# amazon-science/tubelet-transformer

Measured on AMD Instinct MI355X. Metric: clips/sec (TubeR CSN-152 AVA2.1 training step fwd+bwd+clip+AdamW, 32x256x340 clips; whole job), higher is better.
Workload: dtype bf16; 1 GPU; TubeR_CSN152_AVA21 train step, 2 clips/GPU of 3x32x256x340, dropout on, random-init name-hashed weights; global_batch=2, parallelism=dp1, launch_mode=hipgraph, lib_md5=ed8e0d92b699

## Files before the change

### include/tuber_hip.h

```cpp
#ifndef TUBER_HIP_H
#define TUBER_HIP_H

#ifdef __cplusplus
extern "C" {
#endif

typedef struct ihipStream_t* hipStream_t;

typedef struct TuberClipDesc {
    long long src_off;
    int H, W;
    int y1, x1, h, w;
    int flip, jitter;
    int hue, sat, val;
    int pad_;
} TuberClipDesc;

int tuber_attn_fwd(const void* Q, const long* mq, const void* K, const long* mk, const void* V, const long* mv, void* O, const long* mo, float* lse, const void* key_padding_mask, int B, int H, int Lq, int Lk, float scale, float pdrop, const void* seed_ptr, unsigned long long salt, hipStream_t stream);

int tuber_attn_bwd(const void* Q, const long* mq, const void* K, const long* mk, const void* V, const long* mv, const void* O, const long* mo, const float* lse, const void* key_padding_mask, const void* dO, const long* mdo, void* dQ, const long* mdq, void* dK, const long* mdk, void* dV, const long* mdv, float* delta, int B, int H, int Lq, int Lk, float scale, float pdrop, const void* seed_ptr, unsigned long long salt, hipStream_t stream);

int tuber_attn_wide_fwd(const void* q, const void* kv, void* o, int NQ, int HW, int T, float pdrop, const void* seed_ptr, unsigned long long salt, hipStream_t stream);

int tuber_attn_wide_bwd(const void* q, const void* kv, const void* dO, void* dq, void* dkv, int NQ, int HW, int T, float pdrop, const void* seed_ptr, unsigned long long salt, hipStream_t stream);
// ... 16 lines not shown

const char* tuber_comm_last_error(void);

int tuber_comm_unique_id(void* id128);

int tuber_comm_init(const void* id128, int nranks, int rank, int device, void** comm_out);

int tuber_comm_init_timeout(const void* id128, int nranks, int rank, int device, int timeout_ms, void** comm_out);

int tuber_comm_count(void* comm, int* count_out, int* rank_out);

int tuber_comm_allreduce_sum(void* comm, void* buf, long count, int dtype, hipStream_t stream);

int tuber_comm_allreduce_sum_multi(void* comm, void* const* ptrs, const long* counts, int n, int dtype, hipStream_t stream);

int tuber_comm_destroy(void* comm);

int tuber_conv1_bwd_slabs(long M);

int tuber_conv1_bwd_supported(int cin, int p);

int tuber_conv1_bwd_fused(const void* dz1, const void* c1, const float* cA, const float* cB, const float* cC, const void* w1t, long ldw, const void* R, const void* X, const void* Cm, const void* Cd, void* out, float* st0, float* st1, float* st2, float* slab, long M, hipStream_t stream);

int tuber_conv4_bwd_slabs(long M);

int tuber_conv4_bwd_supported(int c4, int p);

int tuber_conv4_bwd_fused(const void* dz, const void* c4, const void* c3, const void* w4t, long ldw, const float* cA, const float* cB, const float* cC, const float* sc3, const float* sh3, void* dz3, float* st0, float* st1, float* slab, long M, hipStream_t stream);

int tuber_criterion_cost(const float* logits, const float* logits_b, const float* boxes, const float* tboxes, const float* tlabels, const int* tcount, int L, int B, int Q, int C, int Tmax, int ava, float w_class, float w_bbox, float w_giou, float* cost, hipStream_t stream);

int tuber_criterion_loss(const float* logits, const float* logits_b, const float* boxes, const float* tboxes, const float* tlabels, const int* tcount, const int* match, int L, int B, int Q, int C, int Tmax, int ava, float eos, float pos_weight, float* losses, float* g_logits, float* g_logits_b, float* g_bbox, float* g_giou, hipStream_t stream);

int tuber_criterion_scale(const float* g, const float* g_logits, const float* g_logits_b, const float* g_bbox, const float* g_giou, int L, long nl, long nb, long nx, float* gl, float* gb, float* gx, hipStream_t stream);

int tuber_weighted_sum(const float* a, const float* w, int n, float* out, const float* gout, float* out_g, hipStream_t stream);

int tuber_lsap_device(const float* cost, const int* tcount, int* match, int L, int B, int Q, int Tmax, hipStream_t stream);

int tuber_class_error(const float* logits, const int* match, const float* tlabels, int B, int Q, int C, int Tmax, int ava, float* out, hipStream_t stream);

int tuber_targets_pack_max(void);

int tuber_targets_pack(const void* const* boxes, const void* const* labels, const int* sizes, int B, int Tmax, int C, int ava, float* tboxes, float* tlabels, int* tcount, hipStream_t stream);

int tuber_mask_resize(const void* mask, void* out, int B, int H, int W, int h, int w, hipStream_t stream);

int tuber_decoder_coop_supported(int d_model, int nhead, int dim_ff, int batch, int num_queries, int num_layers);

int tuber_decoder_coop_ptrs_per_layer(void);

int tuber_decoder_coop_fwd(const void* const* layer_ptrs, const unsigned long long* layer_salts, int num_layers, const void* qpos, const float* norm_weight, const float* norm_bias, void* hs, const void* kpm, int B, int Q, int Lm, float pdrop, float pattn, const void* seed_ptr, void* sync, hipStream_t stream);

int tuber_dwconv_fwd_stat_rows(int N, int To, int Ho, int Wo);

int tuber_dwconv_bwd_data_stat_rows(int N, int Ti, int Hi, int Wi);

int tuber_dwconv_bwd_weight_blocks(int N, int To, int Ho, int Wo);

int tuber_dwconv_fwd(const void* x, const float* sc, const float* sh, const float* w, void* out, float* st0, float* st1, int N, int Ti, int Hi, int Wi, int To, int Ho, int Wo, int C, int st, int ss, hipStream_t stream);

int tuber_dwconv_bwd_data(const void* gout, const float* w, const void* x, const float* sc, const float* sh, void* dz, float* st0, float* st1, int N, int Ti, int Hi, int Wi, int To, int Ho, int Wo, int C, int st, int ss, hipStream_t stream);

int tuber_dw_wgrad_reduce(const float* partial, float* dw, int R, int C, int accumulate, hipStream_t stream);

int tuber_dwconv_bwd_weight(const void* gout, const void* x, const float* sc, const float* sh, float* partial, float* dw, int accumulate, int N, int Ti, int Hi, int Wi, int To, int Ho, int Wo, int C, int st, int ss, hipStream_t stream);

int tuber_dwconv_tile_blocks(int N, int T, int H, int W, int C);

int tuber_dwconv_tile_wgrad_blocks(int N, int T, int H, int W, int C);

int tuber_dwconv_tile_fwd(const void* x, const float* sc, const float* sh, const float* w, void* out, float* st0, float* st1, int N, int T, int H, int W, int C, hipStream_t stream);

int tuber_dwconv_tile_fwd_bn(const void* x, const float* pst0, const float* pst1, int R, float count, const float* gamma, const float* beta, float* rmean, float* rvar, long long* nbt, float momentum, float eps, float* scale, float* shift, float* mean, float* invstd, const float* w, void* out, float* st0, float* st1, int N, int T, int H, int W, int C, hipStream_t stream);

int tuber_dwconv_tile_fwd_bn_ex(const void* x, const float* pst0, const float* pst1, int R, float count, const float* gamma, const float* beta, float* rmean, float* rvar, long long* nbt, float momentum, float eps, float* scale, float* shift, float* mean, float* invstd, const float* w, void* out, float* st0, float* st1, int N, int T, int H, int W, int C, hipStream_t stream);

int tuber_dwconv_tile_bwd_data(const void* gout, const float* w, const void* x, const float* sc, const float* sh, void* dz, float* st0, float* st1, int N, int T, int H, int W, int C, hipStream_t stream);

int tuber_dwconv_tile_bwd_weight(const void* gout, const void* x, const float* sc, const float* sh, float* partial, float* dw, int accumulate, int N, int T, int H, int W, int C, hipStream_t stream);

int tuber_dwconv_tile_bwd_data_bn(const void* dzu, const void* xu, const float* bst0, const float* bst1, int R, float count, const float* gamma, const float* mean, const float* invstd, float* dgamma, float* dbeta, const float* w, const void* x, const float* sc, const float* sh, void* dz, float* st0, float* st1, int N, int T, int H, int W, int C, hipStream_t stream);

int tuber_dwconv_tile_bwd_weight_bn(const void* dzu, const void* xu, const float* bst0, const float* bst1, int R, float count, const float* gamma, const float* mean, const float* invstd, const void* x, const float* sc, const float* sh, float* partial, float* dw, int accumulate, int N, int T, int H, int W, int C, hipStream_t stream);

int tuber_dwconv_tile_bwd_both_bn(const void* dzu, const void* xu, const float* bst0, const float* bst1, int R, float count, const float* gamma, const float* mean, const float* invstd, float* dgamma, float* dbeta, const float* w, const void* x, const float* sc, const float* sh, void* dz, float* st0, float* st1, float* partial, int N, int T, int H, int W, int C, hipStream_t stream);

int tuber_dwconv_tile_bwd_data_bn_frozen(const void* dzu, const float* bst0, const float* bst1, int R, const float* gamma, const float* mean, const float* invstd, float* dgamma, float* dbeta, const float* w, const void* x, const float* sc, const float* sh, void* dz, float* st0, float* st1, int N, int T, int H, int W, int C, hipStream_t stream);

int tuber_dwconv_tile_bwd_weight_bn_frozen(const void* dzu, const float* gamma, const float* mean, const float* invstd, const void* x, const float* sc, const float* sh, float* partial, float* dw, int accumulate, int N, int T, int H, int W, int C, hipStream_t stream);

int tuber_dwconv_tile_bwd_both_bn_frozen(const void* dzu, const float* bst0, const float* bst1, int R, const float* gamma, const float* mean, const float* invstd, float* dgamma, float* dbeta, const float* w, const void* x, const float* sc, const float* sh, void* dz, float* st0, float* st1, float* partial, int N, int T, int H, int W, int C, hipStream_t stream);

int tuber_cast_f32_bf16(const float* src, void* dst, long n, hipStream_t stream);

int tuber_cast_bf16_f32_scale(const void* src, float* dst, long n, float scale, hipStream_t stream);

int tuber_cast_transpose(const float* W, void* WT, int R, int C, int ldt, hipStream_t stream);

int tuber_rows_gather_sum(const void* in, void* out, int A, int B, int C, int D, long sa, long sb, long sc, long sd, int E, float mul, hipStream_t stream);

int tuber_temporal_max_fwd(const void* x, void* out, void* arg, int B, int T, long hw, int E, hipStream_t stream);

int tuber_temporal_max_bwd(const void* g, const void* arg, void* dx, int B, int T, long hw, int E, hipStream_t stream);

int tuber_axpby(const void* a, const void* b, void* out, long n, float alpha, float beta, hipStream_t stream);
// ... 189 lines not shown
```

### tubelet_transformer_amd/ab.py

```python
import contextlib
import os

KNOWN = {
    "no_wgrad_groups": "one tuber_gemm_tn launch per weight-gradient GEMM instead of the grouped launches (engine.WgradQueue)",
    "immediate_reduce": "second-stage reductions of the weight-gradient partials per call instead of the deferred tuber_multi_reduce",
    "no_join_fusion": "stand-alone block_out_bwd instead of the join backward in the conv1 data-gradient GEMM's epilogue",
    "no_fresh_reduce": "tuber_multi_reduce always reads the gradient window it reduces into (out += sum) instead of overwriting the windows zero_grad has just cleared",
    "no_join_mask": "the join backward reads the lower block's output y for its ReLU mask instead of the bit field tuber_block_out_fwd_mask writes (bit-identical gradients)",
    "no_strided_join_fusion": "gemm + rows_scatter_add + block_out_bwd at the stage boundaries instead of the join GEMM with the strided residual",
    "no_ds_join_fusion": "stand-alone block_out_bwd for the first block of every stage (the join kernels take identity-block joins only)",
    "no_bn_bwd_fa": "BatchNorm backward as finalize + apply launches everywhere (no one-launch form)",
    "no_bn_bwd_fa_after_reduce": "no one-launch BatchNorm backward behind the first-stage row reduction (layer1 / layer2)",
    "no_bn1_in_dw_fwd": "stand-alone tuber_bn_finalize for bn1 instead of finalising it inside the stride-1 depthwise forward kernel",
    "no_bn3_in_dw": "stand-alone bn_bwd_fa for bn3 instead of forming it inside the depthwise backward kernels",
    "no_dw_bwd_one_launch": "depthwise data and weight gradient of a stride-1 block as two launches",
    "no_conv4_bwd_fused": "layer1's conv4 backward on the separate BatchNorm / GEMM kernels",
    "no_conv1_bwd_fused": "layer1's conv1 backward on the separate BatchNorm / GEMM kernels",
    "no_blockout_conv1": "layer1's residual join and the next conv1 as two launches",
    "no_entry_conv": "conv1 and the projection conv of layer1's first block as two GEMMs",
    "no_proj_bwd_fused": "layer1's projection-shortcut backward on the separate kernels",
    "no_stem_bn_in_wgrad": "stand-alone bn_bwd_apply for the stem instead of forming it inside the stem weight-gradient kernel",
    "dw_register_tiled": "the register-tiled depthwise kernels (used for the strided blocks) for every block",
    "no_ln_bwd_fusion": "LayerNorm backward and the data-gradient GEMM of the linear in front of it as two launches (no tuber_ln_bwd_dx)",
    "no_in_proj_dx2": "the few-row data gradients of the decoder (in-projection: x and query_pos; linear1) as tuber_gemm_nt launches instead of tuber_rows_dx2",
    "no_decoder_coop": "the DETR decoder stack as its ~80 separate launches instead of the one cooperative launch (csrc/decoder_coop.hip)",
    "eager_step": "train_tuber_detection without the captured hipGraph step",
    "eval_bf16_stream": "eval forward with the residual streams (block outputs, LayerNorm outputs) stored in bf16 like the training path, instead of the fp32 "
                        "streams of the eval precision mode (round 6; also TUBER_EVAL_PRECISION=bf16_stream)",
    "no_eval_conv4_join": "eval precision mode with conv4 and the residual join of an identity block as two launches (tuber_gemm_nt + tuber_block_out_fwd_f32) "
                          "instead of the join in the GEMM epilogue (tuber_gemm_nt_bn_out; bit-identical outputs)",
    "eval_bf16_decoder": "eval precision mode without the fp32 decoder / heads (csrc/eval_f32.hip): the decoder on the bf16 launch chain with fp32 LayerNorm streams only",
}


def _parse(text):
    names = {t.strip().lower() for t in (text or "").replace(";", ",").split(",") if t.strip()}
    bad = sorted(names - set(KNOWN))
    if bad:
        raise ValueError("TUBER_AB: unknown switch(es) %s; known: %s" % (bad, sorted(KNOWN)))
    return names


_active = _parse(os.environ.get("TUBER_AB"))


def on(name):
    if name not in KNOWN:
        raise KeyError(name)
    return name in _active


def active():
    return sorted(_active)


def eval_fp32_stream():
    return not on("eval_bf16_stream") and os.environ.get("TUBER_EVAL_PRECISION", "fp32_stream") != "bf16_stream"


def eval_class_f32():
    return eval_fp32_stream() and os.environ.get("TUBER_EVAL_PRECISION") == "fp32_class"


@contextlib.contextmanager
def override(*names):
    global _active
    old = _active
    _active = _parse(",".join(names))
    try:
        yield
    finally:
        _active = old
```

### tubelet_transformer_amd/backbone.py

```python
import operator
from typing import NamedTuple

import torch
from torch import nn

from . import ab, lib

BN_EPS = 1e-3
BN_MOM = 0.1
BF = torch.bfloat16
CMAX = 2048
_MOMENTUM = operator.attrgetter("momentum")
_TRAINING = operator.attrgetter("training")


class ResNeXtBottleneck(nn.Module):

    def __init__(self, in_planes, planes, stride=1, temporal_stride=1, down_sample=None, expansion=2):
        super().__init__()
        self.expansion = expansion
        self.conv1 = nn.Conv3d(in_planes, planes, kernel_size=1, bias=False)
        self.bn1 = nn.BatchNorm3d(planes, eps=BN_EPS, momentum=BN_MOM)
        self.conv3 = nn.Conv3d(planes, planes, kernel_size=3, bias=False, stride=(temporal_stride, stride, stride),
                               padding=1, groups=planes)
# ... 27 lines not shown
            self.sigmoid = nn.Sigmoid()
        self._runner = None

    @staticmethod
    def _make_layer(in_planes, planes, blocks, stride, temporal_stride, expansion=4):
        ds = nn.Sequential(
            nn.Conv3d(in_planes, planes * expansion, kernel_size=1, stride=(temporal_stride, stride, stride), bias=False),
            nn.BatchNorm3d(planes * expansion, eps=BN_EPS, momentum=BN_MOM))
        layers = [ResNeXtBottleneck(in_planes, planes, stride, temporal_stride, ds, expansion)]
        for _ in range(1, blocks):
            layers.append(ResNeXtBottleneck(planes * expansion, planes, expansion=expansion))
        return nn.Sequential(*layers)

    def forward(self, x):
        raise RuntimeError("ResNeXt runs through tubelet_transformer_amd.tuber.DETR (needs the model's ParamStore)")


def build_CSN(cfg):
    name = cfg.CONFIG.MODEL.BACKBONE_NAME
    if name == "CSN-152":
        m = ResNeXt([3, 8, 36, 3], cfg.CONFIG.DATA.NUM_CLASSES, cfg.CONFIG.MODEL.LAST_STRIDE, with_out_fc=False)
    elif name == "CSN-50":
        m = ResNeXt([3, 4, 6, 3], cfg.CONFIG.DATA.NUM_CLASSES, cfg.CONFIG.MODEL.LAST_STRIDE, with_out_fc=True)
    elif name == "CSN-TEST":
        m = ResNeXt([2, 2, 2, 2], cfg.CONFIG.DATA.NUM_CLASSES, cfg.CONFIG.MODEL.LAST_STRIDE, with_out_fc=False)
    else:
        raise ValueError("unsupported BACKBONE_NAME %r (CSN-50 / CSN-152)" % name)
    if cfg.CONFIG.MODEL.PRETRAINED:
        from .checkpoint import load_csn_mat
        load_csn_mat(m, cfg.CONFIG.MODEL.PRETRAIN_BACKBONE_DIR, name)
    return m


class _BN:
    __slots__ = ("idx", "mod", "C", "gamma", "beta", "rmean", "rvar", "nbt", "dgamma", "dbeta", "scale", "shift", "mean", "invstd",
                 "cA", "cB", "cC")


class _Block:
    __slots__ = ("cin", "p", "st", "ss", "ds", "off0", "stage", "first", "mod", "w1", "g1", "w1t", "ld1t", "w3", "g3", "w4", "g4", "w4t", "ld4t",
                 "bn1", "bn3", "bn4", "wd", "gd", "wdt", "lddt", "bnd")

    @property
    def strided(self):
        return self.st != 1 or self.ss != 1

    @property
    def c4(self):
        return 4 * self.p


_Saved = NamedTuple("_Saved", [(n, object) for n in ("x", "c1", "c3", "c4", "cd", "y", "geom", "ymask")])
_SavedStem = NamedTuple("_SavedStem", [(n, object) for n in ("clips", "c0", "arg", "geom")])


def _rows(B, geom):
    Ti, Hi, Wi, To, Ho, Wo = geom
    return B * Ti * Hi * Wi, B * To * Ho * Wo


class CSNRunner:

    def __init__(self, body: ResNeXt, prefix: str, store):
        self.body, self.store = body, store
        dev = store.device
        self.dev = dev
        bns = [m for m in body.modules() if isinstance(m, nn.BatchNorm3d)]
        self.scratch = torch.zeros(len(bns), 7, CMAX, dtype=torch.float32, device=dev)
        self._bn_index = {}
        self._bn_rows = []
        self.blocks = []
        self.cut_stages = (3,)
        self.split_hook = None
        self.last_y32 = None
        sp = self.scratch.data_ptr()

        def mk_bn(mod_prefix, mod):
            b = _BN()
            i = len(self._bn_index)
            self._bn_index[mod_prefix] = i
            b.idx, b.mod = i, mod
            f, g = store.flat.data_ptr(), store.gflat.data_ptr()
            ow, ob = store.offsets[mod_prefix + ".weight"], store.offsets[mod_prefix + ".bias"]
            b.C = mod.num_features
            b.gamma, b.beta = f + 4 * ow, f + 4 * ob
            b.dgamma, b.dbeta = g + 4 * ow, g + 4 * ob
            b.rmean, b.rvar, b.nbt = mod.running_mean.data_ptr(), mod.running_var.data_ptr(), mod.num_batches_tracked.data_ptr()
            base = sp + 4 * i * 7 * CMAX
            b.scale, b.shift, b.mean, b.invstd, b.cA, b.cB, b.cC = (base + 4 * k * CMAX for k in range(7))
            self._bn_rows.append((i, b))
            return b

        def wptr(name):
            o = store.offsets[name]
            return store.shadow.data_ptr() + 2 * o, store.flat.data_ptr() + 4 * o, store.gflat.data_ptr() + 4 * o

        def tptr(name):
            toff, N, K, ldt = store.tinfo[name]
            return store.tshadow.data_ptr() + 2 * toff, ldt

        self.stem_w32 = store.flat.data_ptr() + 4 * store.offsets[prefix + "conv1.weight"]
        self.stem_g = store.gflat.data_ptr() + 4 * store.offsets[prefix + "conv1.weight"]
        self.stem_wpad = torch.zeros(64, 512, dtype=BF, device=dev)
        self.stem_bn = mk_bn(prefix + "bn1", body.bn1)
        for li in range(1, 5):
            layer = getattr(body, "layer%d" % li)
# ... 453 lines not shown
            if fuse4:
                S4 = lib.query("tuber_conv4_bwd_slabs", Mout)
                part4, acc4 = self.store.partial("c4f", S4 * C4 * P)
                lib.call("tuber_conv4_bwd_fused", dz, sv.c4, c3, d.w4t, d.ld4t, b4.cA, b4.cB, b4.cC, b3.scale, b3.shift,
                         dz3, s0, s1, part4, Mout)
                self._slab_reduce(part4, acc4, d.g4, C4 * P, S4)
            else:
                lib.gemm_nt(dc4, C4, d.w4t, d.ld4t, dz3, P, Mout, P, C4, epi=2, stat0=s0, stat1=s1, Cm=c3, ldcm=P, m_scale=b3.scale, m_shift=b3.shift)
            frz3 = b3.idx in self._frozen
            sfx = "_frozen" if frz3 else ""
            if fuse3 and frz3:
                bs0, bs1, bR = (None, None, 0) if not f["bn3"] else (s0, s1, R3) if R3 <= self._fa_max else self._stat_rows(s0, s1, R3, P)
                bn3 = (dz3, bs0, bs1, bR, b3.gamma, b3.mean, b3.invstd)
                bn3w = (dz3, b3.gamma, b3.mean, b3.invstd)
            elif fuse3:
                bs0, bs1, bR = (s0, s1, R3) if R3 <= self._fa_max else self._stat_rows(s0, s1, R3, P)
                bn3 = bn3w = (dz3, c3, bs0, bs1, bR, float(Mout), b3.gamma, b3.mean, b3.invstd)
            else:
                dc3 = self._bn_bwd(b3, s0, s1, R3, Mout, dz3, c3, Mout, train=f["bn3"], apply=depth >= 4)
        both = not ab.on("no_dw_bwd_one_launch") and fuse3 and f["w3"] and depth >= 5
        if both:
            R1 = nb = lib.query("tuber_dwconv_tile_blocks", B, Ti, Hi, Wi, P)
            part, acc = self.store.partial("tn", nb * 27 * P)
            s0, s1 = self.ws("st0", R1 * P), self.ws("st1", R1 * P)
            dz1 = torch.empty(Min, P, dtype=BF, device=dev)
            lib.call("tuber_dwconv_tile_bwd_both_bn" + sfx, *bn3, b3.dgamma if f["bn3"] else None, b3.dbeta if f["bn3"] else None,
                     d.w3, c1, b1.scale, b1.shift, dz1, s0, s1, part, B, Ti, Hi, Wi, P)
            self._slab_reduce(part, acc, d.g3, 27 * P, nb, P)
            return dz1, s0, s1, R1
        if f["w3"]:
            nb = lib.query("tuber_dwconv_tile_wgrad_blocks", B, Ti, Hi, Wi, P) if tile else lib.query("tuber_dwconv_bwd_weight_blocks", B, To, Hq, Wq)
            part, acc = self.store.partial("tn", nb * 27 * P)
            if fuse3:
                lib.call("tuber_dwconv_tile_bwd_weight_bn" + sfx, *bn3w, c1, b1.scale, b1.shift, part, d.g3, acc, B, Ti, Hi, Wi, P)
            elif tile:
                lib.call("tuber_dwconv_tile_bwd_weight", dc3, c1, b1.scale, b1.shift, part, d.g3, acc, B, Ti, Hi, Wi, P)
            else:
                lib.call("tuber_dwconv_bwd_weight", dc3, c1, b1.scale, b1.shift, part, d.g3, acc, B, Ti, Hi, Wi, To, Hq, Wq, P, st, ss)
            if acc == 2:
                self._slab_reduce(part, acc, d.g3, 27 * P, nb, P)
        if depth < 5:
            return None
        R1 = lib.query("tuber_dwconv_tile_blocks", B, Ti, Hi, Wi, P) if tile else lib.query("tuber_dwconv_bwd_data_stat_rows", B, Ti, Hi, Wi)
        s0, s1 = self.ws("st0", R1 * P), self.ws("st1", R1 * P)
        if tile and b1.idx in self._frozen and not f["bn1"]:
            s0 = s1 = None
        dz1 = torch.empty(Min, P, dtype=BF, device=dev)
        if fuse3:
            lib.call("tuber_dwconv_tile_bwd_data_bn" + sfx, *bn3, b3.dgamma if f["bn3"] else None, b3.dbeta if f["bn3"] else None,
                     d.w3, c1, b1.scale, b1.shift, dz1, s0, s1, B, Ti, Hi, Wi, P)
        elif tile:
            lib.call("tuber_dwconv_tile_bwd_data", dc3, d.w3, c1, b1.scale, b1.shift, dz1, s0, s1, B, Ti, Hi, Wi, P)
        else:
            lib.call("tuber_dwconv_bwd_data", dc3, d.w3, c1, b1.scale, b1.shift, dz1, s0, s1, B, Ti, Hi, Wi, To, Hq, Wq, P, st, ss)
        return dz1, s0, s1, R1

    def _bwd_bn1(self, d, sv, f, depth, need_dx, B, dw):
        Min, _ = _rows(B, sv.geom)
        g1, fuse1 = None, False
        if dw is not None:
            dz1, s0, s1, R1 = dw
            fuse1 = (not ab.on("no_conv1_bwd_fused") and need_dx and not (d.ds and d.strided)
                     and lib.query("tuber_conv1_bwd_supported", d.cin, d.p) == 1)
            dc1 = self._bn_bwd(d.bn1, s0, s1, R1, Min, dz1, sv.c1, Min, train=f["bn1"], apply=depth >= 6 and not fuse1)
            g1 = dz1 if fuse1 else dc1
        if f["w1"] and not fuse1:
            self._wgrad(g1, d.p, sv.x, d.cin, d.g1, Min, d.p, d.cin)
        return g1, fuse1

    def _bwd_shortcut(self, d, sv, f, need_dx, B, join, dcd, fuse_proj):
        dz = join[0]
        cin, C4, x = d.cin, d.c4, sv.x
        Ti, Hi, Wi, To, Hq, Wq = sv.geom
        _, Mout = _rows(B, sv.geom)
        if d.ds and f["wd"] and not fuse_proj:
            gather = (To, Hq, Wq, Ti, Hi, Wi, d.st, d.ss) if d.strided else None
            self._wgrad(dcd, C4, x, cin, d.gd, Mout, C4, cin, 0, None, None, gather)
        if not need_dx or not d.ds:
            return (dz if need_dx else None), None
        dxd = torch.empty(Mout, cin, dtype=BF, device=self.dev)
        if fuse_proj:
            bd = d.bnd
            Sd = lib.query("tuber_conv4_bwd_slabs", Mout)
            partd, accd = self.store.partial("cdf", Sd * C4 * cin)
            lib.call("tuber_conv4_bwd_fused", dz, sv.cd, x, d.wdt, d.lddt, bd.cA, bd.cB, bd.cC, None, None, dxd, None, None, partd, Mout)
            self._slab_reduce(partd, accd, d.gd, C4 * cin, Sd)
        else:
            lib.gemm_nt(dcd, C4, d.wdt, d.lddt, dxd, cin, Mout, cin, C4)
        return (None if d.strided else dxd), dxd

    def _bwd_conv1(self, d, sv, f, B, lower, g1, fuse1, res, dxd):
        cin, P, st, ss, b1, x = d.cin, d.p, d.st, d.ss, d.bn1, sv.x
        Ti, Hi, Wi, To, Hq, Wq = sv.geom
        Min, Mout = _rows(B, sv.geom)
        lb, ls = lower or (None, None)
        strided_ds = d.ds and d.strided
        fuse = not ab.on("no_join_fusion") and lb is not None and not lb.ds and not strided_ds
        fuse_sr = (not ab.on("no_join_fusion") and not ab.on("no_strided_join_fusion") and lb is not None and not lb.ds
                   and strided_ds and not fuse1 and Min % (Ti * Hi * Wi) == 0)
        fuse_ds = (not ab.on("no_join_fusion") and not ab.on("no_ds_join_fusion") and lb is not None and lb.ds
                   and not strided_ds)
        if fuse1:
            part1 = None
            if f["w1"]:
                S1 = lib.query("tuber_conv1_bwd_slabs", Min)
                part1, acc1 = self.store.partial("c1f", S1 * P * cin)
# ... 78 lines not shown
```

### tubelet_transformer_amd/csrc/dwconv.hip

```cpp
#include "common.h"

struct DwGeom { int N, Ti, Hi, Wi, To, Ho, Wo, C, st, ss; };

__device__ __forceinline__ void load_w_chunk(float (*wl)[64], const float* __restrict__ w, int c0, int C) {
    for (int i = threadIdx.x; i < 27 * 64; i += 256) {
        const int tap = i >> 6, c = i & 63;
        wl[tap][c] = (c0 + c < C) ? w[(long)(c0 + c) * 27 + tap] : 0.f;
    }
}

template <int SS>
__global__ __launch_bounds__(256) void dwconv_fwd_kernel(
    const bf16* __restrict__ x, const float* __restrict__ sc, const float* __restrict__ sh, const float* __restrict__ w,
    bf16* __restrict__ out, float* __restrict__ st0, float* __restrict__ st1, DwGeom g, int iters) {
    constexpr int NIN = 3 * SS + 3;
    __shared__ __attribute__((aligned(16))) float wl[27][64];
    __shared__ float red[2][16][64];
    const int cl = threadIdx.x & 15, ps = threadIdx.x >> 4;
    const int c0 = blockIdx.y * 64, c = c0 + cl * 4;
    load_w_chunk(wl, w, c0, g.C);
    float a4[4] = {1.f, 1.f, 1.f, 1.f}, b4[4] = {0.f, 0.f, 0.f, 0.f};
    if (sc) {
        const float4 s = *(const float4*)(sc + c), h = *(const float4*)(sh + c);
        a4[0] = s.x; a4[1] = s.y; a4[2] = s.z; a4[3] = s.w; b4[0] = h.x; b4[1] = h.y; b4[2] = h.z; b4[3] = h.w;
    }
    __syncthreads();
    const int Wg = (g.Wo + 3) >> 2;
    const long segs = (long)g.N * g.To * g.Ho * Wg;
    float s0[4] = {0.f, 0.f, 0.f, 0.f}, s1[4] = {0.f, 0.f, 0.f, 0.f};
    for (int it = 0; it < iters; ++it) {
        const long seg = ((long)blockIdx.x * iters + it) * 16 + ps;
        if (seg >= segs) break;
        const int sg32 = (int)seg;
        int wg = sg32 % Wg; int r = sg32 / Wg;
        const int ho = r % g.Ho; r /= g.Ho;
        const int to = r % g.To; const int n = r / g.To;
        const int wo0 = wg * 4;
        float acc[4][4];
#pragma unroll
        for (int j = 0; j < 4; ++j)
#pragma unroll
            for (int e = 0; e < 4; ++e) acc[j][e] = 0.f;
        uint2 raw[9][NIN];
        unsigned okr = 0;
        int wok = 0;
#pragma unroll
        for (int i = 0; i < NIN; ++i) { const int wi = wo0 * SS - 1 + i; wok |= (wi >= 0 && wi < g.Wi) ? (1 << i) : 0; }
#pragma unroll
        for (int r = 0; r < 9; ++r) {
            const int dt = r / 3, dh = r % 3;
            const int ti = to * g.st + dt - 1, hi = ho * SS + dh - 1;
            const bool ok = ti >= 0 && ti < g.Ti && hi >= 0 && hi < g.Hi;
            okr |= ok ? (1u << r) : 0u;
// ... 242 lines not shown
                        for (int e = 0; e < 4; ++e) acc[tap][e] = fmaf(gv[j][e], in[j * SS + dw][e], acc[tap][e]);
                }
            }
        }
    }
    const int wave = threadIdx.x >> 6;
#pragma unroll
    for (int t = 0; t < 27; ++t)
#pragma unroll
        for (int e = 0; e < 4; ++e) {
            float v = acc[t][e];
            v = xor32_sum(xor16_sum(v));
            if ((threadIdx.x & 63) < 16) red[wave][t][cl * 4 + e] = v;
        }
    __syncthreads();
    for (int i = threadIdx.x; i < 27 * 64; i += 256) {
        const int tap = i >> 6, cc = i & 63;
        if (c0 + cc < g.C)
            P[((long)blockIdx.x * 27 + tap) * g.C + c0 + cc] = red[0][tap][cc] + red[1][tap][cc] + red[2][tap][cc] + red[3][tap][cc];
    }
}

__global__ __launch_bounds__(1024) void dw_wgrad_reduce_kernel(const float* __restrict__ P, float* __restrict__ out, int R, int C, int accumulate) {
    __shared__ float red[32][33];
    const int cl = threadIdx.x & 31, rg = threadIdx.x >> 5;
    const int i = blockIdx.x * 32 + cl;
    const int n = 27 * C;
    float a = 0.f;
    if (i < n) for (int r = rg; r < R; r += 32) a += P[(long)r * n + i];
    red[rg][cl] = a;
    __syncthreads();
    if (rg == 0 && i < n) {
        a = 0.f;
#pragma unroll
        for (int k = 0; k < 32; ++k) a += red[k][cl];
        float* o = out + (long)(i % C) * 27 + i / C;
        *o = accumulate ? *o + a : a;
    }
}

static int dw_blocks(long segs, int* iters, int max_blocks = 4096) {
    long groups = (segs + 15) / 16;
    int it = (int)((groups + max_blocks - 1) / max_blocks);
    if (it < 1) it = 1;
    *iters = it;
    return (int)((groups + it - 1) / it);
}
static const int DW_WGRAD_BLOCKS = 512;

extern "C" {

static bool dw_ok(int C, int st, int ss) { return (C & 63) == 0 && (st == 1 || st == 2) && (ss == 1 || ss == 2); }

int tuber_dwconv_fwd_stat_rows(int N, int To, int Ho, int Wo) {
    int it;
    return dw_blocks((long)N * To * Ho * ((Wo + 3) / 4), &it);
}
int tuber_dwconv_bwd_data_stat_rows(int N, int Ti, int Hi, int Wi) {
    int it;
    return dw_blocks((long)N * Ti * Hi * ((Wi + 3) / 4), &it);
}
int tuber_dwconv_bwd_weight_blocks(int N, int To, int Ho, int Wo) {
    int it;
    return dw_blocks((long)N * To * Ho * ((Wo + 3) / 4), &it, DW_WGRAD_BLOCKS);
}

int tuber_dwconv_fwd(const void* x, const float* sc, const float* sh, const float* w, void* out, float* st0, float* st1,
                     int N, int Ti, int Hi, int Wi, int To, int Ho, int Wo, int C, int st, int ss, hipStream_t stream) {
    if (!dw_ok(C, st, ss)) return TUBER_EINVAL;
    DwGeom g{N, Ti, Hi, Wi, To, Ho, Wo, C, st, ss};
    int iters;
    const int nb = dw_blocks((long)N * To * Ho * ((Wo + 3) / 4), &iters);
    dim3 grid(nb, C / 64), block(256);
    if (ss == 1) hipLaunchKernelGGL(dwconv_fwd_kernel<1>, grid, block, 0, stream, (const bf16*)x, sc, sh, w, (bf16*)out, st0, st1, g, iters);
    else hipLaunchKernelGGL(dwconv_fwd_kernel<2>, grid, block, 0, stream, (const bf16*)x, sc, sh, w, (bf16*)out, st0, st1, g, iters);
    TUBER_RETURN_LAUNCH();
}

int tuber_dwconv_bwd_data(const void* gout, const float* w, const void* x, const float* sc, const float* sh, void* dz,
                          float* st0, float* st1, int N, int Ti, int Hi, int Wi, int To, int Ho, int Wo, int C, int st, int ss,
                          hipStream_t stream) {
    if (!dw_ok(C, st, ss)) return TUBER_EINVAL;
    DwGeom g{N, Ti, Hi, Wi, To, Ho, Wo, C, st, ss};
    int iters;
    const int nb = dw_blocks((long)N * Ti * Hi * ((Wi + 3) / 4), &iters);
    dim3 grid(nb, C / 64), block(256);
    if (ss == 1) hipLaunchKernelGGL(dwconv_bwd_data_kernel<1>, grid, block, 0, stream, (const bf16*)gout, w, (const bf16*)x, sc, sh, (bf16*)dz, st0, st1, g, iters);
    else hipLaunchKernelGGL(dwconv_bwd_data_kernel<2>, grid, block, 0, stream, (const bf16*)gout, w, (const bf16*)x, sc, sh, (bf16*)dz, st0, st1, g, iters);
    TUBER_RETURN_LAUNCH();
}

int tuber_dw_wgrad_reduce(const float* partial, float* dw, int R, int C, int accumulate, hipStream_t stream) {
    hipLaunchKernelGGL(dw_wgrad_reduce_kernel, dim3(ceil_div(27 * C, 32)), dim3(1024), 0, stream, partial, dw, R, C, accumulate);
    TUBER_RETURN_LAUNCH();
}

int tuber_dwconv_bwd_weight(const void* gout, const void* x, const float* sc, const float* sh, float* partial, float* dw,
                            int accumulate, int N, int Ti, int Hi, int Wi, int To, int Ho, int Wo, int C, int st, int ss,
                            hipStream_t stream) {
    if (!dw_ok(C, st, ss)) return TUBER_EINVAL;
    DwGeom g{N, Ti, Hi, Wi, To, Ho, Wo, C, st, ss};
    int iters;
    const int nb = dw_blocks((long)N * To * Ho * ((Wo + 3) / 4), &iters, DW_WGRAD_BLOCKS);
    dim3 grid(nb, C / 64), block(256);
    if (ss == 1) hipLaunchKernelGGL(dwconv_bwd_weight_kernel<1>, grid, block, 0, stream, (const bf16*)gout, (const bf16*)x, sc, sh, partial, g, iters);
    else hipLaunchKernelGGL(dwconv_bwd_weight_kernel<2>, grid, block, 0, stream, (const bf16*)gout, (const bf16*)x, sc, sh, partial, g, iters);
    if (accumulate != 2)
        hipLaunchKernelGGL(dw_wgrad_reduce_kernel, dim3(ceil_div(27 * C, 32)), dim3(1024), 0, stream, partial, dw, nb, C, accumulate);
    TUBER_RETURN_LAUNCH();
}

}
```

### tubelet_transformer_amd/csrc/gen_header.py

```python
import glob
import os
import re

HERE = os.path.dirname(os.path.abspath(__file__))
ROOT = os.path.dirname(os.path.dirname(HERE))

DOC = {
    "tuber_gemm_nt_addproj": "packed attention in-projection with the positional embedding folded in: C = f(A).B^T + bias with f(A) = A + A2 for the output "
                             "columns [0, add_ncols) (q / k rows of in_proj_weight: with_pos_embed, models/transformer/transformer.py:150-159,215-240) and "
                             "f(A) = A for the v rows -- one GEMM instead of an add kernel and two GEMM launches. add_ncols % 128 == 0.",
    "tuber_bn_bwd_fa": "tuber_bn_bwd_finalize + tuber_bn_bwd_apply in ONE launch for short partial lists (layer3 / layer4 of the CSN body): every workgroup "
                       "derives the coefficients of its 128-channel strip from the R partial rows (fp64) and applies dx = cA*dz + cB*x + cC to its rows; "
                       "dgamma / dbeta accumulated by the first row chunk (NULL: frozen BatchNorm). autograd of nn.BatchNorm3d (ir_CSN_152.py:46,56,64,154).",
    "tuber_bn_bwd_fa_max_rows": "largest R tuber_bn_bwd_fa accepts.",
    "tuber_bn_frozen_affine_multi": "the FROZEN BatchNorm layers of a training-mode forward (nn.BatchNorm3d with module.training == False inside model.train(): "
                                    "F.batch_norm(training=False), models/backbones/ir_CSN_152.py:46,56,64,119,154) in ONE launch over a device table of "
                                    "{gamma, beta, running_mean, running_var, scale, shift, mean, invstd, cA, cB, cC, C} rows: scale / shift bit-identical to "
                                    "tuber_bn_eval_affine, mean = running_mean, invstd = 1 / sqrt(running_var + eps), and the backward coefficients cA = gamma * invstd, "
                                    "cB = cC = 0, so every backward kernel that takes (cA, cB, cC) runs unchanged. The running buffers are not written.",
    "tuber_bn_frozen_param_grads": "dgamma += sum dz * (x - running_mean) * invstd, dbeta += sum dz of a frozen BatchNorm whose affine parameters train (autograd of "
                                   "F.batch_norm(training=False), ir_CSN_152.py:46,56,64,119,154) from the partial rows (sum dz, sum dz*x) of the train-mode path: "
                                   "no count, no coefficient output.",
    "tuber_bn_bwd_fa_frozen": "tuber_bn_bwd_fa for a frozen BatchNorm: dx = gamma * invstd * dz in one launch (autograd of F.batch_norm(training=False), "
                              "ir_CSN_152.py:46,56,64,154); x is not an operand, the partial rows are read only for dgamma / dbeta (NULL: not at all).",
# ... 140 lines not shown
    "tuber_dwconv_tile_bwd_data_bn": "tuber_dwconv_tile_bwd_data with the BatchNorm backward of bn3 (autograd of nn.BatchNorm3d, ir_CSN_152.py:56,76-77) folded into its "
                                     "gradient operand: takes bn3's masked output gradient dzu, bn3's input xu (= c3) and the R <= 128 partial rows (sum dz, sum dz*x) "
                                     "instead of a finished dc3; every workgroup derives cA / cB / cC of its 64 channels (fp64) and forms dc3 = cA*dzu + cB*xu + cC "
                                     "in fp32 while staging. dgamma / dbeta of bn3 are accumulated (+=) unless NULL. Replaces tuber_bn_bwd_fa + tuber_dwconv_tile_bwd_data.",
    "tuber_dwconv_tile_bwd_both_bn": "data gradient AND weight gradient of one stride-1 depthwise conv (bn3's backward folded in) in ONE launch and ONE pass over the "
                                     "operands: both are sums over the same (p, p - off) position pairs, so the ring of dc3 staged for the data gradient also feeds "
                                     "dW[off] = sum_p relu(bn1(x))[p] * dc3[p - off] -- 4 tensor passes (read dzu, xu, x; write dz). dz / dgamma / dbeta bit-identical to "
                                     "tuber_dwconv_tile_bwd_data_bn, statistics rows and weight gradient equal up to fp32 summation order; partial = "
                                     "tuber_dwconv_tile_blocks(...) blocks of [27][C], reduced by the caller. autograd of models/backbones/ir_CSN_152.py:48-56,74-77.",
    "tuber_dwconv_tile_bwd_weight_bn": "tuber_dwconv_tile_bwd_weight with the same fold: the output-position gradient is formed from (dzu, xu, partial rows) on load.",
    "tuber_comm_init_timeout": "tuber_comm_init with a deadline: the bootstrap (a collective) runs on a helper thread and the call returns -3 with a message naming "
                               "the waiting rank when its peers have not arrived after timeout_ms -- a dead rank fails the job loudly instead of hanging it "
                               "(what torch.distributed's process-group timeout does for the reference, pipelines/launch.py:44-49). timeout_ms <= 0: no deadline.",
    "tuber_comm_count": "ncclCommCount / ncclCommUserRank of the communicator: the world size and rank RCCL itself sees (rank_out may be NULL).",
    "tuber_cast_bf16_f32_scale": "dst = float(src) * scale: expands a bf16-compressed, all-reduced gradient window back into the fp32 gradient buffer and averages it in the same pass.",
    "tuber_frames_resize": "PIL.Image.resize((nw, nh)) of every decoded frame (datasets/ava_frame.py:146-150; jhmdb_frame.py alike): Pillow's 8-bit two-pass "
                           "fixed-point bicubic (libImaging/Resample.c), packed RGB uint8 [nimg][H][W][3] -> [nimg][Ho][Wo][3], bit-exact.",
    "tuber_clip_prepare": "hflip + crop + ColorJitter + ToTensor/Normalize (datasets/video_transforms.py:69-85,20-66,333-369,308-322; pipeline "
                          "datasets/ava_frame.py:158-176) and the batch collate of utils/misc.py:279-282,367-425 in one pass: uint8 frames -> "
                          "fp32 [N][3][T][Hmax][Wmax] zero padded + bool mask [N][Hmax][Wmax]. One TuberClipDesc per clip (56 bytes: long long src_off; "
                          "int H, W, y1, x1, h, w, flip, jitter, hue, sat, val, pad).",
    "tuber_clip_desc_bytes": "sizeof(TuberClipDesc) as the library was compiled (host-side layout check).",
    "tuber_multi_reduce": "every deferred second-stage reduction of one backward pass in one launch: the weight-gradient launchers called with "
                          "accumulate = 2 (tuber_gemm_tn, tuber_dwconv_*_bwd_weight, tuber_colsum, tuber_layernorm_bwd) leave their partials in place; "
                          "table = MultiReduceEntry[] {const float* P; float* out; long n, stride; int S, mode, C, next}: out[j] += sum_s P[s*stride+j] "
                          "(mode 0 / 2: per element / per float4, s ascending; mode 1: 32-way tree; C > 0: depthwise [S][27][C] -> [C][27]; next: chained contribution to the same out); blk = int2[] (head entry, block in entry), "
                          "1024 / 4096 / 32 elements per block in mode 0 / 2 / 1. Same summation order as the immediate kernels.",
    "tuber_multi_reduce_entry_bytes": "sizeof(MultiReduceEntry) as compiled (host-side layout check).",
    "tuber_temporal_max_fwd": "nn.MaxPool3d((T,1,1)) over the T frames of the backbone features, TEMPORAL_DS_STRATEGY 'max' (models/backbone_builder.py:45-47,73): "
                              "rows (b,t,p) of E bf16 -> rows (b,p) + the uint8 index of the first maximal frame (arg may be NULL in eval).",
    "tuber_temporal_max_bwd": "backward of tuber_temporal_max_fwd: the gradient goes to the frame that held the maximum, zeros elsewhere.",
    "tuber_gemm_nt": "C[M,N] = f(A)[M,K] . B[N,K]^T on MFMA bf16. Replaces every nn.Conv3d(k=1) of the CSN bottlenecks "
                     "(models/backbones/ir_CSN_152.py:41,58,155-161), input_proj/class_proj (models/tuber_ava.py:57-58) and every "
                     "nn.Linear / packed in-projection (models/transformer/transformer.py:159-165,227-245; transformer_layers.py:81-94; "
                     "tuber_ava.py:65-71), plus their data gradients (B = W^T). amode 1 fuses relu(x*a_scale[k]+a_shift[k]) "
                     "(BatchNorm apply, ir_CSN_152.py:72-79) into the A load; gather=1 reads A rows through the strided "
                     "(n,t*st,h*ss,w*ss) map of the down_sample conv (:155-161). epi 0: +bias, +R, ReLU, bf16|fp32 out; "
                     "epi 1: bf16 out + per-column partial (sum, sum^2) rows for training-mode BatchNorm; epi 2: out = acc*[Cm*m_scale+m_shift>0] "
                     "+ partial (sum dz, sum dz*Cm) rows for BatchNorm backward (stat rows optional: with m_scale NULL it is the ReLU / ReLU+Dropout "
                     "backward mask from the saved activation). Accumulators are scaled by alpha first; epi 0 can end with Dropout(drop_p) "
                     "keyed by (seed, salt, m*N+n) -- FFN linear1 (transformer.py:160-162). K % 64 == 0.",
    "tuber_gemm_nt_cfg": "tile configuration tuber_gemm_nt uses for (M,N,K): 13 = 64x64 (two-tile prefetch), 7 = 64x128, 0 = 128x128 (plain epilogue only); 2 / 12 / 17 = rejected A/B variants, built only with -DTUBER_AB_VARIANTS.",
    "tuber_gemm_tn_tile": "output tile edge of the transpose-read weight-gradient kernel for (M, N, K): 128 (mid-M backbone shapes, N and K multiples of 128) or 64.",
    "tuber_gemm_nt_has_cfg": "1 when tuber_gemm_nt_set_cfg(cfg) names a tile configuration this library was built with.",
    "tuber_gemm_nt_stat_rows": "rows of partial statistics tuber_gemm_nt(epi 1|2) writes for (M,N).",
    "tuber_gemm_tn": "dW[N,K] (+)= sum_m G[m,N]^T . f(A)[m,K]: weight gradient of the same convs / linears (autograd of the ops above); "
                     "split over M into fp32 slabs `partial` [tuber_gemm_tn_slabs][N][K], then reduced deterministically.",
    "tuber_gemm_tn_fuses_bias": "can tuber_gemm_tn also produce the bias gradient for this shape: 0 no; 1 yes, accumulated into bias_grad[N] directly (single slab); 2 yes, bias_grad receives one partial row per slab ([tuber_gemm_tn_slabs][N], reduced by the caller).",
    "tuber_gemm_tn_slabs": "number of slabs (size of `partial` / (N*K)) tuber_gemm_tn uses.",
    "tuber_dwconv_fwd": "depthwise Conv3d(C,C,3,groups=C,stride=(st,ss,ss),padding=1) on NDHWC bf16, ResNeXtBottleneck.conv3 "
                        "(ir_CSN_152.py:48-51) with relu(bn1(.)) fused on load (sc/sh may be NULL) and bn3 partial statistics on store.",
    "tuber_dwconv_bwd_data": "input gradient of conv3 fused with the backward of relu(bn1(.)): dz = da*[x*sc+sh>0] + partial (sum dz, sum dz*x).",
    "tuber_dwconv_bwd_weight": "weight gradient of conv3 ([C][27] fp32), activation relu(bn1(x)) recomputed on load.",
    "tuber_dwconv_fwd_stat_rows": "partial-stat rows written by tuber_dwconv_fwd.",
    "tuber_dwconv_bwd_data_stat_rows": "partial-stat rows written by tuber_dwconv_bwd_data.",
    "tuber_dwconv_bwd_weight_blocks": "blocks (size of `partial` / (27*C)) used by tuber_dwconv_bwd_weight.",
    "tuber_dwconv_tile_fwd_bn": "tuber_bn_finalize + tuber_dwconv_tile_fwd in ONE launch: the training-mode BatchNorm in front of conv3 (bn1, ir_CSN_152.py:46-51) is "
                                "finalised inside the conv -- every workgroup derives scale / shift of its 64 channels from the producing conv's R partial rows "
                                "(pst0 = sum x, pst1 = sum x^2 over `count` rows; fp64 sums, the arithmetic of tuber_bn_finalize expression for expression), the first "
                                "workgroup of each channel group writes scale / shift / mean / invstd [C] and updates rmean / rvar / nbt (NULL: none). Other arguments as tuber_dwconv_tile_fwd.",
    "tuber_dwconv_tile_fwd_bn_ex": "tuber_dwconv_tile_fwd_bn with the momentum contract of tuber_bn_finalize_ex: the module's momentum as given, or (momentum < 0) "
                                   "the cumulative average of nn.BatchNorm3d(momentum=None) with nbt read, not written (tuber_bn_count_advance). "
                                   "reference: ir_CSN_152.py:46-51 under torch.optim.swa_utils.update_bn.",
    "tuber_dwconv_tile_fwd": "stride-1 conv3 (ir_CSN_152.py:48-51) with the input planes staged once per workgroup in an LDS ring (activated on the way in): "
                             "same contract as tuber_dwconv_fwd for st = ss = 1; partial-stat rows = tuber_dwconv_tile_blocks.",
    "tuber_dwconv_tile_bwd_data": "LDS-staged data gradient of the stride-1 conv3, fused with the backward of relu(bn1(.)) like tuber_dwconv_bwd_data.",
    "tuber_dwconv_tile_bwd_weight": "LDS-staged weight gradient of the stride-1 conv3 (activation recomputed while staging).",
    "tuber_dwconv_tile_blocks": "workgroups along x of the LDS-staged depthwise kernels = partial-stat rows / weight-gradient partial blocks.",
    "tuber_dwconv_tile_wgrad_blocks": "partial blocks (size of `partial` / (27*C)) of tuber_dwconv_tile_bwd_weight.",
    "tuber_dw_wgrad_reduce": "dw[c][tap] (+)= sum_r partial[r][tap][c]: second stage of the depthwise weight gradient.",
    "tuber_bn_finalize": "training-mode nn.BatchNorm3d(eps=1e-3, momentum=0.1) statistics (ir_CSN_152.py:15-16,46,56,64,119,154): partial rows -> "
                         "mean/invstd, scale=gamma*invstd, shift=beta-mean*scale, running_mean/var (unbiased) and num_batches_tracked update.",
    "tuber_bn_finalize_ex": "tuber_bn_finalize with the module's momentum as given (nn.BatchNorm3d.momentum, ir_CSN_152.py:15-16,46,56,64,119,154; "
                            "running = (1 - m) * running + m * batch, num_batches_tracked += 1). momentum < 0 selects the cumulative average of "
                            "momentum=None (torch.nn.modules.batchnorm._BatchNorm.forward): m = 1 / (n + 1) with n = *num_batches_tracked read on the device, "
                            "which this launch leaves unchanged so that every workgroup sees the same n -- tuber_bn_count_advance increments it after the forward.",
    "tuber_bn_count_advance": "num_batches_tracked += 1 (the `self.num_batches_tracked.add_(1)` of _BatchNorm.forward under momentum=None) for every BatchNorm "
                              "of a DEVICE table of n int64 counter addresses, in ONE launch: the layers finalised in cumulative mode by tuber_bn_finalize_ex / "
                              "tuber_dwconv_tile_fwd_bn_ex during the forward.",
    "tuber_stat_rows_reduce": "first stage for long partial-statistics lists (R > 512 rows: layer1): [R][C] x2 -> [tuber_stat_rows_reduced(R)][C] x2.",
    "tuber_stat_rows_reduced": "rows left by tuber_stat_rows_reduce (R itself when no first stage is needed).",
    "tuber_bn_eval_affine": "eval-mode BatchNorm3d folded to scale/shift from the running statistics.",
    "tuber_bn_bwd_finalize": "BatchNorm backward coefficients: dx = cA*dz + cB*x + cC, dgamma = sum dz*xhat, dbeta = sum dz.",
    "tuber_bn_bwd_apply": "dx = cA*dz + cB*x + cC (BatchNorm backward apply), bf16 [M,C].",
    "tuber_block_out_fwd": "bottleneck join y = relu(bn4(c4) + shortcut) (ir_CSN_152.py:81-90); shortcut = res or bn_ds(res) when rs/rh given.",
    "tuber_block_out_bwd": "backward of the join: dz = dy*[y>0] and the partial statistics of bn4 (and of the down_sample BN).",
    "tuber_rowblock_count": "partial-stat rows written by the row-blocked reduce kernels for M rows.",
    "tuber_layernorm_fwd": "y = LayerNorm(Dropout_p(x) (+ res)) over E in {256, 2048}, eps 1e-5 (nn.LayerNorm, transformer.py:163-167,229-247,116-123; "
                           "transformer_layers.py:84,91,96,437-445); saves xhat (bf16) and rstd for backward.",
    "tuber_layernorm_bwd": "backward of tuber_layernorm_fwd: dx (gradient of res), dxd (gradient of x through the regenerated dropout mask) and dgamma/dbeta via block partials.",
    "tuber_layernorm_bwd_blocks": "blocks used by tuber_layernorm_bwd (partial = 2*blocks*E floats).",
    "tuber_reduce_rows": "out[c] (+)= sum_r P[r][c].",
    "tuber_colsum_blocks": "row blocks (size of `partial` / C) used by tuber_colsum.",
    "tuber_colsum": "bias gradient: out[c] (+)= sum_m g[m][c] for bf16 g.",
    "tuber_gemm_nt_set_cfg": "tuning hook: force tile configuration cfg for every later tuber_gemm_nt (-1 = automatic choice).",
    "tuber_stem_conv_fwd": "stem Conv3d(3,64,(3,7,7),s=(1,2,2),p=(1,3,3)) (ir_CSN_152.py:109-115) as an implicit MFMA GEMM from the fp32 NCDHW clip to NDHWC bf16, "
                           "with the partial statistics of the following BatchNorm; Wp = tuber_stem_pack_weight(conv1.weight).",
    "tuber_stem_conv_bwd_weight": "weight gradient of the stem conv ([64][441] fp32) as an implicit MFMA GEMM (no patch matrix in HBM).",
    "tuber_stem_conv_blocks": "persistent grid size of the stem conv forward = its partial-stat rows.",
    "tuber_stem_conv_wgrad_blocks": "workgroups (= [512][64] fp32 partial slabs) of tuber_stem_conv_bwd_weight.",
    "tuber_stem_pack_weight": "conv1.weight [64][441] fp32 -> [64][512] bf16 with k' = (c,kt,kh)*8 + kw (zero padded).",
    "tuber_stem_pool_fwd": "relu(bn1(.)) + MaxPool3d((1,3,3),s=(1,2,2),p=(0,1,1)) (ir_CSN_152.py:119-122) on NDHWC bf16, C=64; saves the argmax tap.",
    "tuber_stem_pool_bwd": "backward of the pool + relu(bn1(.)): dz and the BN-backward partial statistics.",
    "tuber_stem_pool_bwd_stat_rows": "partial-stat rows written by tuber_stem_pool_bwd.",
    "tuber_attn_fwd": "softmax(scale*QK^T + key_padding_mask)[dropout] V for 32-wide heads, operands read in place through strided token maps "
                      "{ld,sL,s1,s2,B2}: row(l,b) = l*sL + (b/B2)*s1 + (b%B2)*s2. Core of nn.MultiheadAttention "
# ... 133 lines not shown
```

Baseline: 147.1 clips/s.

## Add LDS-staged depthwise data-gradient kernel for spatially strided stage-entry blocks

Adds a new kernel for the input gradient of the stride-2 depthwise conv3 at stage entries. It stages output-gradient planes in a four-plane LDS ring and keeps the weight slice in LDS, so each input position reuses the staged gradients instead of re-reading them from global memory. The kernel is the default, with an A/B switch back to the register-tiled kernel. It risks LDS pressure and lower occupancy, and the statistics rows are summed in a different order.

```diff
diff --git a/include/tuber_hip.h b/include/tuber_hip.h
--- a/include/tuber_hip.h
+++ b/include/tuber_hip.h
@@ -92,6 +92,8 @@
 
 int tuber_decoder_coop_fwd(const void* const* layer_ptrs, const unsigned long long* layer_salts, int num_layers, const void* qpos, const float* norm_weight, const float* norm_bias, void* hs, const void* kpm, int B, int Q, int Lm, float pdrop, float pattn, const void* seed_ptr, void* sync, hipStream_t stream);
 
+int tuber_dwconv_strided_lds_set(int on);
+
 int tuber_dwconv_fwd_stat_rows(int N, int To, int Ho, int Wo);
 
 int tuber_dwconv_bwd_data_stat_rows(int N, int Ti, int Hi, int Wi);
diff --git a/tubelet_transformer_amd/ab.py b/tubelet_transformer_amd/ab.py
--- a/tubelet_transformer_amd/ab.py
+++ b/tubelet_transformer_amd/ab.py
@@ -21,6 +21,7 @@
     "no_proj_bwd_fused": "layer1's projection-shortcut backward on the separate kernels",
     "no_stem_bn_in_wgrad": "stand-alone bn_bwd_apply for the stem instead of forming it inside the stem weight-gradient kernel",
     "dw_register_tiled": "the register-tiled depthwise kernels (used for the strided blocks) for every block",
+    "dw_strided_register_tiled": "the register-tiled depthwise data-gradient kernel for the spatially strided stage-entry blocks instead of the LDS-staged one (csrc/dwconv_strided.hip)",
     "no_ln_bwd_fusion": "LayerNorm backward and the data-gradient GEMM of the linear in front of it as two launches (no tuber_ln_bwd_dx)",
     "no_in_proj_dx2": "the few-row data gradients of the decoder (in-projection: x and query_pos; linear1) as tuber_gemm_nt launches instead of tuber_rows_dx2",
     "no_decoder_coop": "the DETR decoder stack as its ~80 separate launches instead of the one cooperative launch (csrc/decoder_coop.hip)",
diff --git a/tubelet_transformer_amd/backbone.py b/tubelet_transformer_amd/backbone.py
--- a/tubelet_transformer_amd/backbone.py
+++ b/tubelet_transformer_amd/backbone.py
@@ -103,6 +103,10 @@
 
 _Saved = NamedTuple("_Saved", [(n, object) for n in ("x", "c1", "c3", "c4", "cd", "y", "geom", "ymask")])
 _SavedStem = NamedTuple("_SavedStem", [(n, object) for n in ("clips", "c0", "arg", "geom")])
+
+
+def _dw_strided_switch():
+    lib.query("tuber_dwconv_strided_lds_set", 0 if ab.on("dw_strided_register_tiled") else 1)
 
 
 def _rows(B, geom):
@@ -662,6 +666,7 @@
         elif tile:
             lib.call("tuber_dwconv_tile_bwd_data", dc3, d.w3, c1, b1.scale, b1.shift, dz1, s0, s1, B, Ti, Hi, Wi, P)
         else:
+            _dw_strided_switch()
             lib.call("tuber_dwconv_bwd_data", dc3, d.w3, c1, b1.scale, b1.shift, dz1, s0, s1, B, Ti, Hi, Wi, To, Hq, Wq, P, st, ss)
         return dz1, s0, s1, R1
 
diff --git a/tubelet_transformer_amd/csrc/dwconv.hip b/tubelet_transformer_amd/csrc/dwconv.hip
--- a/tubelet_transformer_amd/csrc/dwconv.hip
+++ b/tubelet_transformer_amd/csrc/dwconv.hip
@@ -1,4 +1,8 @@
 #include "common.h"
+
+bool dwconv_strided_bwd_data(const void* gout, const float* w, const void* x, const float* sc, const float* sh, void* dz,
+                             float* st0, float* st1, int N, int Ti, int Hi, int Wi, int To, int Ho, int Wo, int C, int st, int R,
+                             hipStream_t stream);
 
 struct DwGeom { int N, Ti, Hi, Wi, To, Ho, Wo, C, st, ss; };
 
@@ -347,6 +351,9 @@
 
 static bool dw_ok(int C, int st, int ss) { return (C & 63) == 0 && (st == 1 || st == 2) && (ss == 1 || ss == 2); }
 
+static int g_dw_strided_lds = 1;
+int tuber_dwconv_strided_lds_set(int on) { g_dw_strided_lds = on; return 0; }
+
 int tuber_dwconv_fwd_stat_rows(int N, int To, int Ho, int Wo) {
     int it;
     return dw_blocks((long)N * To * Ho * ((Wo + 3) / 4), &it);
@@ -380,6 +387,8 @@
     int iters;
     const int nb = dw_blocks((long)N * Ti * Hi * ((Wi + 3) / 4), &iters);
     dim3 grid(nb, C / 64), block(256);
+    if (ss == 2 && g_dw_strided_lds && dwconv_strided_bwd_data(gout, w, x, sc, sh, dz, st0, st1, N, Ti, Hi, Wi, To, Ho, Wo, C, st, nb, stream))
+        TUBER_RETURN_LAUNCH();
     if (ss == 1) hipLaunchKernelGGL(dwconv_bwd_data_kernel<1>, grid, block, 0, stream, (const bf16*)gout, w, (const bf16*)x, sc, sh, (bf16*)dz, st0, st1, g, iters);
     else hipLaunchKernelGGL(dwconv_bwd_data_kernel<2>, grid, block, 0, stream, (const bf16*)gout, w, (const bf16*)x, sc, sh, (bf16*)dz, st0, st1, g, iters);
     TUBER_RETURN_LAUNCH();
diff --git a/tubelet_transformer_amd/csrc/dwconv_strided.hip b/tubelet_transformer_amd/csrc/dwconv_strided.hip
--- /dev/null
+++ b/tubelet_transformer_amd/csrc/dwconv_strided.hip
@@ -0,0 +1,163 @@
+#include "common.h"
+
+#ifndef DWS_CAP_DATA
+#define DWS_CAP_DATA 3072
+#endif
+
+namespace {
+
+struct SGeom {
+    int N, Ti, Hi, Wi, To, Ho, Wo, C;
+    int tc, tchunks, htiles, wtiles;
+    int G, R;
+};
+
+__device__ __forceinline__ void load_w_slice(float* wl, const float* __restrict__ w, int c0) {
+    for (int i = threadIdx.x; i < 27 * 64; i += 256) wl[(i % 27) * 64 + i / 27] = w[(long)c0 * 27 + i];
+}
+
+__device__ __forceinline__ void tile_of(const SGeom& g, int b, int& n, int& tk, int& ht, int& wt) {
+    wt = b % g.wtiles; b /= g.wtiles;
+    ht = b % g.htiles; b /= g.htiles;
+    tk = b % g.tchunks; n = b / g.tchunks;
+}
+
+constexpr int GPH = 3, GPW = 9, GNPOS = GPH * GPW;
+constexpr int GSTR = 96;
+
+template <int ST>
+__global__ __launch_bounds__(256) void dwconv_strided_bwd_data_kernel(
+    const bf16* __restrict__ gout, const float* __restrict__ w, const bf16* __restrict__ x, const float* __restrict__ sc,
+    const float* __restrict__ sh, bf16* __restrict__ dz, float* __restrict__ st0, float* __restrict__ st1, SGeom g) {
+    __shared__ __attribute__((aligned(16))) bf16 ring[4][GNPOS * GSTR];
+    __shared__ __attribute__((aligned(16))) float wl[27 * 64];
+    __shared__ float red[2][16][64];
+    const int tid = threadIdx.x, cl = tid & 15, ps = tid >> 4, row = ps >> 2, cg = ps & 3;
+    const int bx = xcd_remap(blockIdx.x, gridDim.x);
+    const int c0 = blockIdx.y * 64, c = c0 + cl * 4;
+    int n, tk, ht, wt;
+    tile_of(g, bx, n, tk, ht, wt);
+    const int h0 = ht * 4, w0 = wt * 16, t0 = tk * g.tc, t1 = min(g.Ti, t0 + g.tc);
+    load_w_slice(wl, w, c0);
+    float a4[4], b4[4];
+    {
+        const float4 s = *(const float4*)(sc + c), h = *(const float4*)(sh + c);
+        a4[0] = s.x; a4[1] = s.y; a4[2] = s.z; a4[3] = s.w; b4[0] = h.x; b4[1] = h.y; b4[2] = h.z; b4[3] = h.w;
+    }
+    const int spos = tid >> 3, sq = tid & 7;
+    const int sho = h0 / 2 + spos / GPW, swo = w0 / 2 + spos % GPW;
+    const bool s_in = spos < GNPOS;
+    const bool s_ok = s_in && sho < g.Ho && swo < g.Wo;
+    const long s_off = s_ok ? ((long)sho * g.Wo + swo) * g.C + c0 + sq * 8 : 0;
+    const long gplane = (long)g.Ho * g.Wo * g.C;
+    const bf16* gn = gout + (long)n * g.To * gplane;
+    const int hi = h0 + row, wi0 = w0 + cg * 4;
+    const bool row_in = hi < g.Hi;
+    float s0[4] = {0.f, 0.f, 0.f, 0.f}, s1[4] = {0.f, 0.f, 0.f, 0.f};
+    int loaded = max((t0 - 1 + ST - 1) / ST, 0) - 1;
+    for (int ti = t0; ti < t1; ++ti) {
+        const long pos = (((long)n * g.Ti + ti) * g.Hi + min(hi, g.Hi - 1)) * (long)g.Wi;
+        uint2 xr[4];
+#pragma unroll
+        for (int j = 0; j < 4; ++j) xr[j] = *(const uint2*)(x + (pos + min(wi0 + j, g.Wi - 1)) * g.C + c);
+        const int need = min((ti + 1) / ST, g.To - 1);
+        while (loaded < need) {
+            ++loaded;
+            if (s_in) {
+                uint4 v = *(const uint4*)(gn + (long)loaded * gplane + s_off);
+                if (!s_ok) v = make_uint4(0u, 0u, 0u, 0u);
+                *(uint4*)(&ring[loaded & 3][spos * GSTR + sq * 8]) = v;
+            }
+        }
+        __syncthreads();
+        float acc[4][4];
+#pragma unroll
+        for (int j = 0; j < 4; ++j)
+#pragma unroll
+            for (int e = 0; e < 4; ++e) acc[j][e] = 0.f;
+#pragma unroll
+        for (int r = 0; r < 9; ++r) {
+            const int dt = r / 3, dh = r % 3;
+            const int tn = ti + 1 - dt, hn = hi + 1 - dh;
+            const int to = tn / ST, ho = hn / 2;
+            const bool ok = tn >= 0 && (tn % ST) == 0 && to < g.To && hn >= 0 && (hn % 2) == 0 && ho < g.Ho;
+            if (!ok) continue;
+            const bf16* rp = &ring[to & 3][((ho - h0 / 2) * GPW + cg * 2) * GSTR + cl * 4];
+            float gw[3][4];
+#pragma unroll
+            for (int i = 0; i < 3; ++i) {
+                const bf16x4 v = as_bf16x4(*(const uint2*)(rp + i * GSTR));
+#pragma unroll
+                for (int e = 0; e < 4; ++e) gw[i][e] = bf2f(v[e]);
+            }
+#pragma unroll
+            for (int dw = 0; dw < 3; ++dw) {
+                const float4 wv = *(const float4*)&wl[(r * 3 + dw) * 64 + cl * 4];
+                const float ww[4] = {wv.x, wv.y, wv.z, wv.w};
+#pragma unroll
+                for (int j = 0; j < 4; ++j) {
+                    const int num = j + 1 - dw;
+                    if (num >= 0 && (num & 1) == 0) {
+#pragma unroll
+                        for (int e = 0; e < 4; ++e) acc[j][e] = fmaf(gw[num >> 1][e], ww[e], acc[j][e]);
+                    }
+                }
+            }
+        }
+        if (row_in) {
+#pragma unroll
+            for (int j = 0; j < 4; ++j) {
+                if (wi0 + j < g.Wi) {
+                    const bf16x4 xv = as_bf16x4(xr[j]);
+                    bf16x4 o;
+#pragma unroll
+                    for (int e = 0; e < 4; ++e) {
+                        const float xf = bf2f(xv[e]);
+                        const float v = fmaf(xf, a4[e], b4[e]) > 0.f ? acc[j][e] : 0.f;
+                        o[e] = f2bf(v);
+                        s0[e] += v; s1[e] += v * xf;
+                    }
+                    *(uint2*)(dz + (pos + wi0 + j) * g.C + c) = as_uint2(o);
+                }
+            }
+        }
+    }
+#pragma unroll
+    for (int e = 0; e < 4; ++e) { red[0][ps][cl * 4 + e] = s0[e]; red[1][ps][cl * 4 + e] = s1[e]; }
+    __syncthreads();
+    if (tid < 128) {
+        const int which = tid >> 6, cc = tid & 63;
+        float a = 0.f;
+#pragma unroll
+        for (int s = 0; s < 16; ++s) a += red[which][s][cc];
+        float* dst = which ? st1 : st0;
+        dst[(long)bx * g.C + c0 + cc] = a;
+        for (int r = g.G + bx; r < g.R; r += g.G) dst[(long)r * g.C + c0 + cc] = 0.f;
+    }
+}
+
+bool tile_grid(SGeom& g, int planes, int th, int tw, int H, int W, int cap, int R) {
+    g.htiles = ceil_div(H, th);
+    g.wtiles = ceil_div(W, tw);
+    g.R = R;
+    for (int tc = 1; tc <= planes; ++tc) {
+        g.tc = tc;
+        g.tchunks = ceil_div(planes, tc);
+        g.G = g.N * g.tchunks * g.htiles * g.wtiles;
+        if (g.G <= R && ((long)g.G * (g.C / 64) <= cap || tc == planes)) return true;
+    }
+    return false;
+}
+
+}
+
+bool dwconv_strided_bwd_data(const void* gout, const float* w, const void* x, const float* sc, const float* sh, void* dz,
+                             float* st0, float* st1, int N, int Ti, int Hi, int Wi, int To, int Ho, int Wo, int C, int st, int R,
+                             hipStream_t stream) {
+    SGeom g{N, Ti, Hi, Wi, To, Ho, Wo, C};
+    if (!tile_grid(g, Ti, 4, 16, Hi, Wi, DWS_CAP_DATA, R)) return false;
+    dim3 grid(g.G, C / 64), block(256);
+    if (st == 1) hipLaunchKernelGGL(dwconv_strided_bwd_data_kernel<1>, grid, block, 0, stream, (const bf16*)gout, w, (const bf16*)x, sc, sh, (bf16*)dz, st0, st1, g);
+    else hipLaunchKernelGGL(dwconv_strided_bwd_data_kernel<2>, grid, block, 0, stream, (const bf16*)gout, w, (const bf16*)x, sc, sh, (bf16*)dz, st0, st1, g);
+    return true;
+}
diff --git a/tubelet_transformer_amd/csrc/gen_header.py b/tubelet_transformer_amd/csrc/gen_header.py
--- a/tubelet_transformer_amd/csrc/gen_header.py
+++ b/tubelet_transformer_amd/csrc/gen_header.py
@@ -216,6 +216,9 @@
                         "(ir_CSN_152.py:48-51) with relu(bn1(.)) fused on load (sc/sh may be NULL) and bn3 partial statistics on store.",
     "tuber_dwconv_bwd_data": "input gradient of conv3 fused with the backward of relu(bn1(.)): dz = da*[x*sc+sh>0] + partial (sum dz, sum dz*x).",
     "tuber_dwconv_bwd_weight": "weight gradient of conv3 ([C][27] fp32), activation relu(bn1(x)) recomputed on load.",
+    "tuber_dwconv_strided_lds_set": "A/B switch and test hook: 0 sends the spatially strided calls (ss == 2) of tuber_dwconv_bwd_data back to the register-tiled "
+                                    "kernel, 1 (default) runs the LDS-staged kernel of csrc/dwconv_strided.hip: bit-identical dz, statistics rows equal up to fp32 "
+                                    "summation order, the same row count.",
     "tuber_dwconv_fwd_stat_rows": "partial-stat rows written by tuber_dwconv_fwd.",
     "tuber_dwconv_bwd_data_stat_rows": "partial-stat rows written by tuber_dwconv_bwd_data.",
     "tuber_dwconv_bwd_weight_blocks": "blocks (size of `partial` / (27*C)) used by tuber_dwconv_bwd_weight.",
```

After: 147.5 clips/s, median of 6. About the same (+0.3%).
